# avi2924/Speech-Intent-Recognizer

Measured on AMD Instinct MI355X. Metric: utterances/sec (16 kHz, 3 s clips), inference: HIP STFT+mel+CNN/BiGRU forward + argmax, higher is better.
Workload: dtype f32

## Files before the change

devtools/kernel_ab/legacy_kernels.h:

```cpp
#pragma once
#include "../csrc/bf16x6_kernels.h"

constexpr int XB_ROW = 80;

constexpr int conv_bf16x6_row_bytes(int PC, bool pad = true) {
    const int slots = (4 * PC + 2) * 3;
    return (pad ? slots + ((4 - slots % 8) + 8) % 8 : slots) * 16;
}
constexpr size_t conv_bf16x6_lds_bytes(int PR, int PC, bool pad = true) { return (size_t)3 * (8 * PR + 2) * conv_bf16x6_row_bytes(PC, pad); }


static __global__ __launch_bounds__(256) void gemm_nt_bf16x6_kernel(
    const unsigned short* __restrict__ Ap, const unsigned short* __restrict__ Bp0, const unsigned short* __restrict__ Bp1,
    const float* __restrict__ bias0, const float* __restrict__ bias1, float* __restrict__ C, int ldc, int M, int N, int K) {
    __shared__ __attribute__((aligned(16))) unsigned char As[3 * GB_M * XB_ROW];
    __shared__ __attribute__((aligned(16))) unsigned char Bs[3 * GB_N * XB_ROW];
    const int z = blockIdx.z;
    const unsigned short* __restrict__ Bp = z ? Bp1 : Bp0;
    const float* __restrict__ bias = z ? bias1 : bias0;
    const int m0 = blockIdx.y * GB_M, n0 = blockIdx.x * GB_N;
    const int tid = threadIdx.x, lane = tid & 63, wv = tid >> 6;
    const int wm = wv >> 1, wn = wv & 1, m = lane & 31, h = lane >> 5;
    const size_t planeA = (size_t)M * K, planeB = (size_t)N * K;

// ... 227 lines not shown
                    if (PYb + q < Hp) out[(((size_t)b * Hp + PYb + q) * Wp + PX) * COUT + co] = pooled[q];
            } else {
                float* o = out + ((size_t)b * Wp + PX) * (COUT * Hp) + (size_t)co * Hp + PYb;
                if ((Hp & 3) == 0) {
                    *reinterpret_cast<float4*>(o) = make_float4(pooled[0], pooled[1], pooled[2], pooled[3]);
                } else {
#pragma unroll
                    for (int q = 0; q < 4; ++q)
                        if (PYb + q < Hp) o[q] = pooled[q];
                }
            }
        }
    }
}

static __global__ __launch_bounds__(256) void split3_kernel(const float* __restrict__ in, int ld_in, unsigned short* __restrict__ out,
                                                             size_t rows, int K) {
    split3_rows(in, ld_in, out, rows, K, (size_t)blockIdx.x * 256 + threadIdx.x, (size_t)gridDim.x * 256);
}


constexpr int G3_BM = 160, G3_BN = 256, G3_BK = 32;
constexpr int G3_APLANE = G3_BM * 64, G3_BPLANE = G3_BN * 64;
constexpr int G3_BOFF = 3 * G3_APLANE;
constexpr int G3_STAGE = G3_BOFF + 3 * G3_BPLANE;
constexpr int G3_LDS_BYTES = 2 * G3_STAGE;
constexpr int G3_APIECES = 3 * G3_BM / 16, G3_PIECES = G3_APIECES + 3 * G3_BN / 16;
constexpr int G3_DEFAULT = 16;

template <int KNOCK = G3_DEFAULT>
static __global__ __launch_bounds__(512) void gemm_nt_bf16x6_v3_kernel(
    const unsigned short* __restrict__ Ap, const unsigned short* __restrict__ Bp0, const unsigned short* __restrict__ Bp1,
    const float* __restrict__ bias0, const float* __restrict__ bias1, float* __restrict__ C, int ldc, int M, int N, int K) {
    extern __shared__ __attribute__((aligned(1024))) unsigned char g3_smem[];
    const int nwg = gridDim.x, orig = blockIdx.x, xcd = orig & 7, q = nwg >> 3, rem = nwg & 7;
    const int wgid = (xcd < rem ? xcd * (q + 1) : rem * (q + 1) + (xcd - rem) * q) + (orig >> 3);
    const int nbd = N / G3_BN, nb = 2 * nbd;
    const int mblk = wgid / nb, nbk = wgid - mblk * nb, z = nbk / nbd;
    const int m0 = mblk * G3_BM, n0 = (nbk - z * nbd) * G3_BN;
    const unsigned short* __restrict__ Bp = z ? Bp1 : Bp0;
    const float* __restrict__ bias = z ? bias1 : bias0;
    const int tid = threadIdx.x, lane = tid & 63, wv = tid >> 6, m = lane & 31, h = lane >> 5;
    const size_t planeA = (size_t)M * K, planeB = (size_t)N * K;

    const int lr = lane >> 2;
    const int csrc = (lane & 3) ^ ((lr >> 2) & 3);
    unsigned int poff[10];
#pragma unroll
    for (int i = 0; i < 10; ++i) {
        const int g = wv + 8 * i;
        if (g < G3_APIECES) {
            const int pl = g / 10, rg = g - pl * 10;
            int row = m0 + rg * 16 + lr;
            row = row < M ? row : M - 1;
            poff[i] = (unsigned int)(pl * planeA + (size_t)row * K + csrc * 8);
        } else {
            const int gb = g - G3_APIECES, pl = gb >> 4, rg = gb & 15;
            poff[i] = (unsigned int)(pl * planeB + (size_t)(n0 + rg * 16 + lr) * K + csrc * 8);
        }
    }
    auto piece = [&](int i, int kt, int buf) {
        if (KNOCK & 1) return;
        const int g = wv + 8 * i;
        if (g < G3_PIECES) {
            const unsigned short* src = (g < G3_APIECES ? Ap : Bp) + poff[i] + (size_t)kt * G3_BK;
            __builtin_amdgcn_global_load_lds((sir_gptr_t)src, (sir_lptr_t)(g3_smem + buf * G3_STAGE + g * 1024), 16, 0, 0);
        }
    };
    auto stage = [&](int kt, int buf) {
#pragma unroll
        for (int i = 0; i < 10; ++i) piece(i, kt, buf);
    };

    f32x16 acc[5];
#pragma unroll
    for (int mt = 0; mt < 5; ++mt)
#pragma unroll
        for (int r = 0; r < 16; ++r) acc[mt][r] = 0.0f;

    int fo[2];
#pragma unroll
    for (int ks = 0; ks < 2; ++ks) fo[ks] = m * 64 + ((((ks << 1) | h) ^ ((m >> 2) & 3)) << 4);

    constexpr int SPREAD = (KNOCK >> 3) & 3;
    constexpr bool PREF = (KNOCK >> 5) & 1;
    const int nk = K / G3_BK;
    bf16x8 a[2][3][5], bb[2][3];
    auto read_frags = [&](int buf, int ks) {
        const unsigned char* abase = g3_smem + buf * G3_STAGE;
        const unsigned char* bbase = abase + G3_BOFF + wv * 2048;
#pragma unroll
        for (int p = 0; p < 3; ++p) {
            bb[ks][p] = __builtin_bit_cast(bf16x8, *reinterpret_cast<const uint4*>(bbase + p * G3_BPLANE + fo[ks]));
#pragma unroll
            for (int mt = 0; mt < 5; ++mt)
                a[ks][p][mt] = __builtin_bit_cast(bf16x8, *reinterpret_cast<const uint4*>(abase + p * G3_APLANE + mt * 2048 + fo[ks]));
        }
    };
    auto compute = [&](int buf, int ktn) {
        const int ktl = ktn < nk ? ktn : nk - 1;
        read_frags(buf, 0);
        if (PREF) {
            read_frags(buf, 1);
            __builtin_amdgcn_sched_barrier(0);
        }
#pragma unroll
        for (int ks = 0; ks < 2; ++ks) {
            if (!PREF && ks == 1) read_frags(buf, 1);
            constexpr int PA[6] = {2, 0, 1, 1, 0, 0}, PB[6] = {0, 2, 1, 0, 1, 0};
#pragma unroll
            for (int t = 0; t < 6; ++t)
#pragma unroll
                for (int mt = 0; mt < 5; ++mt) {
                    if (KNOCK & 4) acc[mt][0] += __builtin_bit_cast(float4, a[ks][PA[t]][mt]).x * __builtin_bit_cast(float4, bb[ks][PB[t]]).x;
                    else acc[mt] = __builtin_amdgcn_mfma_f32_32x32x16_bf16(a[ks][PA[t]][mt], bb[ks][PB[t]], acc[mt], 0, 0, 0);
                    const int idx = t * 5 + mt;
                    if (SPREAD && idx % 3 == 2) {
                        if (SPREAD == 1 && ks == 0) piece(idx / 3, ktl, buf ^ 1);
                        if (SPREAD == 2 && ks == (wv >> 2)) piece(idx / 3, ktl, buf ^ 1);
                    }
                }
        }
    };

    stage(0, 0);
    for (int kt = 0; kt < nk; ++kt) {
        __syncthreads();
        if (SPREAD == 0 && kt + 1 < nk) stage(kt + 1, (kt + 1) & 1);
        compute(kt & 1, kt + 1);
    }

    const int n = n0 + wv * 32 + m;
    const float bv = bias ? bias[n] : 0.0f;
    float* crow = C + (size_t)(m0 + 4 * h) * ldc + (size_t)z * N + n;
    if (m0 + G3_BM <= M) {
#pragma unroll
        for (int mt = 0; mt < 5; ++mt)
#pragma unroll
            for (int r = 0; r < 16; ++r) crow[(size_t)(mt * 32 + (r & 3) + 8 * (r >> 2)) * ldc] = acc[mt][r] + bv;
    } else {
#pragma unroll
        for (int mt = 0; mt < 5; ++mt)
#pragma unroll
            for (int r = 0; r < 16; ++r) {
                const int ro = mt * 32 + (r & 3) + 8 * (r >> 2);
                if (m0 + 4 * h + ro < M) crow[(size_t)ro * ldc] = acc[mt][r] + bv;
            }
    }
}

static inline bool gemm_bf16x6_v3_ok(int M, int N, int K) {
    return N % G3_BN == 0 && K % G3_BK == 0 && (size_t)3 * M * K < ((size_t)1 << 31) && (size_t)3 * N * K < ((size_t)1 << 31);
}
```

speech-intent-recognizer_amd/csrc/model_infer.hip:

```cpp
#include "f16x3_kernels.h"
#include "conv_fwd.h"
#include "infer_tables.h"

extern "C" size_t sir_model_workspace_bytes(const sir_handle* h, int batch, int t_frames, int train) {
    (void)h;
    if (train) return sir_train_workspace_bytes_impl(batch, t_frames);
    Dims d;
    if (!make_dims(batch, t_frames, &d)) return 0;
    size_t off[WS_COUNT];
    return iws_layout(d, off);
}

extern "C" int sir_model_workspace_offsets(const sir_handle* h, int batch, int t_frames, int train, size_t* offsets,
                                           int n) {
    (void)h; (void)train;
    Dims d;
    if (!make_dims(batch, t_frames, &d) || !offsets) {
        sir_set_error("sir_model_workspace_offsets: bad shape batch=%d t_frames=%d (need " SIR_SHAPE_LIMITS ")", batch, t_frames);
        return SIR_EINVAL;
    }
    size_t off[WS_COUNT];
    iws_layout(d, off);
    for (int i = 0; i < n && i < WS_COUNT; ++i) offsets[i] = off[i];
    return WS_COUNT;
}

extern "C" int sir_model_infer_table_offsets(const sir_handle* h, int batch, int t_frames, size_t* offsets, int n) {
    (void)h;
    Dims d;
    if (!make_dims(batch, t_frames, &d) || !offsets) {
        sir_set_error("sir_model_infer_table_offsets: bad shape batch=%d t_frames=%d (need " SIR_SHAPE_LIMITS ")", batch, t_frames);
        return SIR_EINVAL;
    }
    const ITabs t = itab_layout(d);
    const size_t v[] = {t.e0, t.d1, t.d3, t.rows, t.tab2, t.tab3, t.record, t.nonfinite, t.count, (size_t)WS_PAD};
    const int nv = (int)(sizeof(v) / sizeof(v[0]));
    for (int i = 0; i < n && i < nv; ++i) offsets[i] = v[i];
    return nv;
}

static int model_infer_impl(const char* who, sir_handle* h, const sir_model_weights* w, const float* feats, const int32_t* frames, int batch,
                            int t_frames, float* logits, int64_t* argmax, void* workspace, size_t workspace_bytes, void* stream_) {
    if (!h || !w || !feats || !logits || !workspace) { sir_set_error("%s: NULL argument", who); return SIR_EINVAL; }
    Dims d;
    if (!make_dims(batch, t_frames, &d)) {
        sir_set_error("%s: unsupported shape batch=%d t_frames=%d (need " SIR_SHAPE_LIMITS ")", who, batch, t_frames);
        return SIR_EINVAL;
    }
    if (h->cfg.n_mels != 64) { sir_set_error("%s: the model is wired for 64 mels (models.py:23)", who); return SIR_EUNSUPPORTED; }
    if (w->num_classes < 1 || w->num_classes > 64) { sir_set_error("%s: num_classes=%d", who, w->num_classes); return SIR_EINVAL; }
    size_t off[WS_COUNT];
    const size_t need = iws_layout(d, off);
    if (workspace_bytes < need) { sir_set_error("%s: workspace %zu < %zu", who, workspace_bytes, need); return SIR_ENOMEM; }
    if (((uintptr_t)workspace & 255) != 0) { sir_set_error("%s: workspace must be 256-byte aligned", who); return SIR_EINVAL; }
    const bool ragged = frames != nullptr;
    hipStream_t st = (hipStream_t)stream_;
    const IPtrs p = carve(workspace, off, d);
    const ITabPtrs& t = p.t;
    const int B = d.B, S = d.S;
    const bool proj_throughput = h->cluster_multi;

    const SirConvPlan cp = sir_conv_plan(&d, true);
    const bool w2 = cp.fwd_wino;
    const int BT = w2 ? B + 1 : B;

    const long long prep_key = ((long long)B << 32) | (unsigned)d.T;
    sir_handle::PrepEntry* pe = nullptr;
    for (auto& e : h->prep)
        if (e.ws == workspace) pe = &e;
    const bool reuse_prep = pe && h->weights_version != 0 && pe->version == h->weights_version && pe->key == prep_key;
    if (!reuse_prep) {
        SirProfScope prof(h, SIR_K_PREP, st);
        const int bn_c[3] = {32, 64, 128}, bn_o[3] = {0, 32, 96};
        for (int i = 0; i < 3; ++i)
            hipLaunchKernelGGL(prep_bn_kernel, dim3(1), dim3(128), 0, st, w->bn_w[i], w->bn_b[i], w->bn_mean[i], w->bn_var[i],
                               p.bns + bn_o[i], p.bnt + bn_o[i], bn_c[i], i == 0 ? w->conv_w[0] : (const float*)nullptr, i == 0 ? 288 : 0, h->status);
        for (int i = 0; i < 4; ++i) sir_prep_whh_quad(h, st, w->gru_w_hh[i], p.whh[i]);
        if (w2) hipLaunchKernelGGL(prep_conv_w_wino_f16x3_kernel, dim3(prep_blocks(WCB_W2)), dim3(256), 0, st, w->conv_w[1], p.wcb2, 32, 64, h->status);
        else hipLaunchKernelGGL(prep_conv_w_wino_bf16x3_kernel, dim3(prep_blocks(WCB_W2)), dim3(256), 0, st, w->conv_w[1], p.wcb2, 32, 64);
        if (w2) hipLaunchKernelGGL(prep_conv_w_wino_f16x3_kernel, dim3(prep_blocks(WCB_W3)), dim3(256), 0, st, w->conv_w[2], p.wcb3, 64, 128, h->status);
        else hipLaunchKernelGGL(prep_conv_w_wino_bf16x3_kernel, dim3(prep_blocks(WCB_W3)), dim3(256), 0, st, w->conv_w[2], p.wcb3, 64, 128);
        hipLaunchKernelGGL(prep_conv_w_bf16x3_kernel, dim3(prep_blocks(WCB_W3_TAPS)), dim3(256), 0, st, w->conv_w[2], p.wcb3d, 64, 128);
        for (int dir = 0; dir < 2; ++dir) {
            hipLaunchKernelGGL(split2h_weights_kernel, dim3(WS_DIR0_BLOCKS), dim3(256), 0, st, w->gru_w_ih[dir], 1024, p.wsl0[dir], (size_t)768, 1024, h->status);
            hipLaunchKernelGGL(split2h_weights_kernel, dim3(WS_DIR1_BLOCKS), dim3(256), 0, st, w->gru_w_ih[2 + dir], 512, p.wsl1[dir], (size_t)768, 512, h->status);
        }
        if (!pe) { pe = &h->prep[h->prep_next]; h->prep_next = (h->prep_next + 1) % 4; }
        pe->ws = workspace; pe->version = h->weights_version; pe->key = prep_key;
    }
    SIR_KCHECK();

    {
        SirProfScope prof(h, SIR_K_CONV1, st);
        hipLaunchKernelGGL(pad_extent_kernel, dim3(B), dim3(256), 0, st, feats, d.T, ragged ? nullptr : t.e0, (const int*)frames, t.nonfinite);
        if (ragged) {
            hipLaunchKernelGGL(ragged_tables_kernel, dim3(1), dim3(1024), 0, st, (const int*)frames, d, t.e0, t.d1, t.d3, t.tab2, t.tab3, t.rows, h->status);
            hipLaunchKernelGGL(conv1_mfma_bn_relu_pool_ragged_kernel, conv1_grid(B, d.wp1), dim3(256), 0, st, feats,
                               w->conv_w[0], p.bns, p.bnt, p.a1, 64, d.T, 32, d.wp1, t.d1, t.e0);
            if (!w2) hipLaunchKernelGGL(ragged_mask_kernel, dim3(32, B), dim3(256), 0, st, p.a1, t.e0, 1, 32, d.wp1, 32);
        } else {
            if (w2) hipLaunchKernelGGL(pad_tables_kernel, dim3(1), dim3(1024), 0, st, t.e0, d, t.d1, t.d3, t.tab2, t.tab3, t.rows, p.xz);
            hipLaunchKernelGGL(conv1_mfma_bn_relu_pool_kernel, conv1_grid(BT, d.wp1), dim3(256), 0, st, feats,
                               w->conv_w[0], p.bns, p.bnt, p.a1, 64, d.T, 32, d.wp1, p.xz, B, w2 ? t.d1 : nullptr);
        }
    }
    {
        SirProfScope prof(h, SIR_K_CONV2, st);
        if (ragged) {
            SIR_TRY((conv_fwd<32, 64, 0, true>(h, st, w2, cp.geo2, B, p.a1, p.wcb2, nullptr, p.bns + 32, p.bnt + 32, p.a2, nullptr, t.tab2, (B + 1) * d.k2max,
                                               t.e0, 1)));
            if (!w2) hipLaunchKernelGGL(ragged_mask_kernel, dim3(16, B), dim3(256), 0, st, p.a2, t.e0, 2, 16, d.wp2, 64);
        } else
            SIR_TRY((conv_fwd<32, 64, 0>(h, st, w2, cp.geo2, BT, p.a1, p.wcb2, nullptr, p.bns + 32, p.bnt + 32, p.a2, nullptr, t.tab2, (B + 1) * d.k2max)));
    }
    {
        SirProfScope prof(h, SIR_K_CONV3, st);
        if (ragged)
            SIR_TRY((conv_fwd<64, 128, 1, true>(h, st, w2, cp.geo3, B, p.a2, p.wcb3, p.wcb3d, p.bns + 96, p.bnt + 96, p.x0, (float2*)p.xs, t.tab3, (B + 1) * d.k3max,
                                                t.e0, 2)));
        else
            SIR_TRY((conv_fwd<64, 128, 1>(h, st, w2, cp.geo3, BT, p.a2, p.wcb3, p.wcb3d, p.bns + 96, p.bnt + 96, p.x0, (float2*)p.xs, t.tab3, (B + 1) * d.k3max)));
    }
    SIR_KCHECK();

    const int M = B * S;
    const int* const nlive0 = w2 || ragged ? t.d3 : nullptr;
    const int* const nlive1 = ragged ? t.d3 : nullptr;
    {
        SirProfScope prof(h, SIR_K_GEMM_IH0, st);
        if (w2 || ragged)
            SIR_TRY(launch_gemm_nt_f16x3_gather(h, st, p.xs, p.wsl0[0], p.wsl0[1], w->gru_b_ih[0], w->gru_b_ih[1], p.gi, 1536,
                                                t.rows, BT * S, 768, 1024, proj_throughput, t.record));
        else
            SIR_TRY(launch_gemm_nt_f16x3(h, st, p.xs, p.wsl0[0], p.wsl0[1], w->gru_b_ih[0], w->gru_b_ih[1], p.gi, 1536, M, 768, 1024));
    }
    {
        SirProfScope prof(h, SIR_K_GRU0, st);
        SIR_TRY(sir_launch_gru_quad(h, st, false, p.gi, w->gru_w_hh[0], w->gru_w_hh[1], w->gru_b_hh[0], w->gru_b_hh[1], p.y0, B, S, nullptr,
                                    p.xs, p.whh[0], p.whh[1], nlive0, ragged));
    }
    {
        SirProfScope prof(h, SIR_K_GEMM_IH1, st);
        if (ragged)
            SIR_TRY(launch_gemm_nt_f16x3_gather(h, st, p.xs, p.wsl1[0], p.wsl1[1], w->gru_b_ih[2], w->gru_b_ih[3], p.gi, 1536,
                                                t.rows, M, 768, 512, proj_throughput, t.record));
        else
            SIR_TRY(launch_gemm_nt_f16x3(h, st, p.xs, p.wsl1[0], p.wsl1[1], w->gru_b_ih[2], w->gru_b_ih[3], p.gi, 1536, M, 768, 512));
    }
    {
        SirProfScope prof(h, SIR_K_GRU1, st);
        SIR_TRY(sir_launch_gru_quad(h, st, false, p.gi, w->gru_w_hh[2], w->gru_w_hh[3], w->gru_b_hh[2], w->gru_b_hh[3], p.y1, B, S, nullptr,
                                    nullptr, p.whh[2], p.whh[3], nlive1, ragged));
    }
    SIR_KCHECK();

    {
        SirProfScope prof(h, SIR_K_ATTN, st);
        if (ragged)
            hipLaunchKernelGGL(attention_pool_ragged_kernel, dim3(B), dim3(256), 0, st, p.y1, w->attn_w, w->attn_b, p.ctx, S, w->fc_w, w->fc_b,
                               w->num_classes, logits, (long long*)argmax, t.d3, t.nonfinite);
        else
            hipLaunchKernelGGL(attention_pool_kernel, dim3(B), dim3(256), 0, st, p.y1, w->attn_w, w->attn_b, p.ctx, S, w->fc_w, w->fc_b,
                               w->num_classes, logits, (long long*)argmax, t.nonfinite, nullptr);
    }
    SIR_KCHECK();
    return SIR_OK;
}

extern "C" int sir_model_infer(sir_handle* h, const sir_model_weights* w, const float* feats, int batch, int t_frames,
                               float* logits, int64_t* argmax, void* workspace, size_t workspace_bytes, void* stream_) {
    return model_infer_impl("sir_model_infer", h, w, feats, nullptr, batch, t_frames, logits, argmax, workspace, workspace_bytes, stream_);
}

extern "C" int sir_model_infer_ragged(sir_handle* h, const sir_model_weights* w, const float* feats, const int32_t* frames, int batch,
                                      int t_frames, float* logits, int64_t* argmax, void* workspace, size_t workspace_bytes,
                                      void* stream_) {
    if (!frames) { sir_set_error("sir_model_infer_ragged: NULL frames"); return SIR_EINVAL; }
    return model_infer_impl("sir_model_infer_ragged", h, w, feats, frames, batch, t_frames, logits, argmax, workspace, workspace_bytes, stream_);
}
```

speech-intent-recognizer_amd/csrc/model_kernels.h:

```cpp
#pragma once
#include "sir_internal.h"
#include "model_shape.h"

typedef float f32x16 __attribute__((ext_vector_type(16)));
typedef float mk_f32x2 __attribute__((ext_vector_type(2)));

#define SIR_BN_EPS 1e-5f


constexpr unsigned int SIR_STATUS_BN_PARAM = 8192u;
__device__ __forceinline__ bool sir_finite(float v) { return fabsf(v) < INFINITY; }
__device__ __forceinline__ void sir_flag_bn_param(bool ok, unsigned int* status) {
    if (!ok) __hip_atomic_fetch_or(status, SIR_STATUS_BN_PARAM, __ATOMIC_RELAXED, __HIP_MEMORY_SCOPE_AGENT);
}

#ifndef SIR_NO_STANDALONE_KERNELS
static __global__ void prep_bn_kernel(const float* __restrict__ g, const float* __restrict__ b, const float* __restrict__ mean,
                               const float* __restrict__ var, float* __restrict__ scale, float* __restrict__ shift, int c,
                               const float* __restrict__ w1, int n1, unsigned int* __restrict__ status) {
    const int i = blockIdx.x * blockDim.x + threadIdx.x;
    if (i >= c) return;
    const float s = g[i] / sqrtf(var[i] + SIR_BN_EPS);
    const float t = b[i] - mean[i] * s;
    scale[i] = s;
    shift[i] = t;
    bool ok = sir_finite(s) && sir_finite(t);
    for (int j = i; j < n1; j += c) ok = ok && sir_finite(w1[j]);
    sir_flag_bn_param(ok, status);
}
#endif

constexpr int C1_PROWS = 4, C1_PCOLS = 32;
constexpr int C1_TR = 2 * C1_PROWS + 2, C1_TC = 2 * C1_PCOLS + 2;
inline dim3 conv1_grid(int images, int Wp) { return dim3(images, 1, (Wp + C1_PCOLS - 1) / C1_PCOLS); }

#ifndef SIR_NO_STANDALONE_KERNELS
template <bool RAGGED>
__device__ __forceinline__ void conv1_mfma_bn_relu_pool_body(
    const float* __restrict__ x, const float* __restrict__ w, const float* __restrict__ scale,
    const float* __restrict__ shift, float* __restrict__ out, int H, int W, int Hp, int Wp,
    const float* __restrict__ xtail, int nx, const int* __restrict__ lim, const int* __restrict__ xlim) {
    __shared__ float tiles[2][C1_TR * C1_TC];
    const int b = blockIdx.x, px0 = blockIdx.z * C1_PCOLS;
    const int wlim = lim ? min(Wp, lim[b]) : Wp;
    if (px0 >= wlim) return;
    const int tid = threadIdx.x, lane = tid & 63, wv = tid >> 6, j = lane & 31, kh = lane >> 5;
    const float* xb = b < nx ? x + (size_t)b * H * W : xtail;
    const int Wx = RAGGED ? min(W, xlim[b]) : W;
    constexpr int NPRE = (C1_TR * C1_TC + 255) / 256;
    float pre[NPRE];
    auto fetch = [&](int py0) {
#pragma unroll
        for (int q = 0; q < NPRE; ++q) {
            const int i = tid + 256 * q, ty = i / C1_TC, tx = i - ty * C1_TC;
            const int gy = 2 * py0 - 1 + ty, gx = 2 * px0 - 1 + tx;
            pre[q] = (i < C1_TR * C1_TC && gy >= 0 && gy < H && gx >= 0 && gx < Wx) ? xb[(size_t)gy * W + gx] : 0.0f;
        }
    };
    fetch(0);
    float wa[5];
    int boff[5];
#pragma unroll
    for (int s = 0; s < 5; ++s) {
        const int tap = 2 * s + kh;
        wa[s] = tap < 9 ? w[j * 9 + tap] : 0.0f;
        const int tc = tap < 9 ? tap : 8;
        boff[s] = (tc / 3) * C1_TC + (tc % 3) + j;
    }
    float sc[16], sh[16];
#pragma unroll
    for (int r = 0; r < 16; ++r) {
        const int ch = (r & 3) + 8 * (r >> 2) + 4 * kh;
        sc[r] = scale[ch]; sh[r] = shift[ch];
    }
    const bool odd = j & 1;
    int it = 0;
    for (int py0 = 0; py0 < Hp; py0 += C1_PROWS, ++it) {
        float* tile = tiles[it & 1];
#pragma unroll
        for (int q = 0; q < NPRE; ++q)
            if (tid + 256 * q < C1_TR * C1_TC) tile[tid + 256 * q] = pre[q];
        __syncthreads();
        if (py0 + C1_PROWS < Hp) fetch(py0 + C1_PROWS);
        const int py = py0 + wv;
        if (py >= Hp) continue;
        const float* trow = tile + (2 * wv) * C1_TC;
#pragma unroll
        for (int h = 0; h < 2; ++h) {
            if (px0 + 16 * h >= wlim) break;
            f32x16 acc0, acc1;
#pragma unroll
            for (int r = 0; r < 16; ++r) { acc0[r] = 0.0f; acc1[r] = 0.0f; }
#pragma unroll
            for (int s = 0; s < 5; ++s) {
                const float b0 = trow[boff[s] + 32 * h], b1 = trow[boff[s] + 32 * h + C1_TC];
                acc0 = __builtin_amdgcn_mfma_f32_32x32x2f32(wa[s], b0, acc0, 0, 0, 0);
                acc1 = __builtin_amdgcn_mfma_f32_32x32x2f32(wa[s], b1, acc1, 0, 0, 0);
            }
            float m[16];
#pragma unroll
            for (int r = 0; r < 16; r += 2) {
                const mk_f32x2 s2 = {sc[r], sc[r + 1]}, h2 = {sh[r], sh[r + 1]};
                const mk_f32x2 y0 = __builtin_elementwise_fma((mk_f32x2){acc0[r], acc0[r + 1]}, s2, h2);
                const mk_f32x2 y1 = __builtin_elementwise_fma((mk_f32x2){acc1[r], acc1[r + 1]}, s2, h2);
                const float v0 = fmaxf(y0.x, y1.x), v1 = fmaxf(y0.y, y1.y);
                const float nb0 = __builtin_bit_cast(float, __builtin_amdgcn_update_dpp(0, __builtin_bit_cast(int, v0), 0xB1, 0xF, 0xF, true));
                const float nb1 = __builtin_bit_cast(float, __builtin_amdgcn_update_dpp(0, __builtin_bit_cast(int, v1), 0xB1, 0xF, 0xF, true));
                m[r] = fmaxf(fmaxf(v0, nb0), 0.0f);
                m[r + 1] = fmaxf(fmaxf(v1, nb1), 0.0f);
            }
            const int px = px0 + 16 * h + (j >> 1);
            const float4 lo = odd ? make_float4(m[8], m[9], m[10], m[11]) : make_float4(m[0], m[1], m[2], m[3]);
            const float4 hi = odd ? make_float4(m[12], m[13], m[14], m[15]) : make_float4(m[4], m[5], m[6], m[7]);
            if (px < wlim) {
                float* o = out + (((size_t)b * Hp + py) * Wp + px) * 32 + 4 * kh + (odd ? 16 : 0);
                *reinterpret_cast<float4*>(o) = lo;
                *reinterpret_cast<float4*>(o + 8) = hi;
            }
        }
    }
}
static __global__ __launch_bounds__(256, 4) void conv1_mfma_bn_relu_pool_kernel(
    const float* __restrict__ x, const float* __restrict__ w, const float* __restrict__ scale,
    const float* __restrict__ shift, float* __restrict__ out, int H, int W, int Hp, int Wp,
    const float* __restrict__ xtail, int nx, const int* __restrict__ lim) {
    conv1_mfma_bn_relu_pool_body<false>(x, w, scale, shift, out, H, W, Hp, Wp, xtail, nx, lim, nullptr);
}
static __global__ __launch_bounds__(256, 4) void conv1_mfma_bn_relu_pool_ragged_kernel(
    const float* __restrict__ x, const float* __restrict__ w, const float* __restrict__ scale,
    const float* __restrict__ shift, float* __restrict__ out, int H, int W, int Hp, int Wp,
    const int* __restrict__ lim, const int* __restrict__ xlim) {
    conv1_mfma_bn_relu_pool_body<true>(x, w, scale, shift, out, H, W, Hp, Wp, nullptr, (int)gridDim.x, lim, xlim);
}
#endif

constexpr int GB_M = 128, GB_N = 64, GB_K = 32, GB_S = GB_K + 4;

constexpr int GRU_H = 256, GRU_BW = 2;
constexpr int GRU_NPART = 4;
constexpr int GRU_KPER4 = 64 / GRU_NPART;
constexpr int GRU_KREG4 = 3;
constexpr int GRU_KLDS4 = 2;
constexpr int GRU_KSTR4 = GRU_KPER4 - GRU_KREG4 - GRU_KLDS4;
constexpr int GRU_NQ = (GRU_BW + GRU_NPART - 1) / GRU_NPART;
constexpr int GRU_THREADS = 256 * GRU_NPART;
constexpr size_t GRU_LDS_BYTES =
    (size_t)(GRU_NPART * GRU_KLDS4 * 3 * 256 * 4 + GRU_BW * GRU_H + GRU_NPART * GRU_BW * 3 * GRU_H) * 4;

__device__ __forceinline__ float sigmoidf_(float x) { return 1.0f / (1.0f + expf(-x)); }

template <int NB>
__device__ __forceinline__ void gru_fma4(float (&acc)[NB], const float4 w, const float4 (&h4)[NB]) {
#pragma unroll
    for (int bb = 0; bb < NB; ++bb) {
        acc[bb] = fmaf(w.x, h4[bb].x, acc[bb]); acc[bb] = fmaf(w.y, h4[bb].y, acc[bb]);
        acc[bb] = fmaf(w.z, h4[bb].z, acc[bb]); acc[bb] = fmaf(w.w, h4[bb].w, acc[bb]);
    }
}


#ifndef SIR_NO_STANDALONE_KERNELS
template <bool RAGGED>
__device__ __forceinline__ void attention_pool_body(const float* __restrict__ y, const float* __restrict__ aw,
                                                    const float* __restrict__ ab, float* __restrict__ ctx,
                                                    int SR, const float* __restrict__ fcw,
                                                    const float* __restrict__ fcb, int C,
                                                    float* __restrict__ logits, long long* __restrict__ amax,
                                                    const int* __restrict__ slen, const int* __restrict__ bad_row,
                                                    const double* __restrict__ sumsq) {
    __shared__ float sc[ATT_MAX_S];
    __shared__ float cs[512];
    __shared__ float lg[64];
    const int b = blockIdx.x, tid = threadIdx.x, lane = tid & 63, wv = tid >> 6;
    const int S = RAGGED ? min(SR, slen[b]) : SR;
    bool bad = bad_row && bad_row[b] != 0;
    if (sumsq) bad |= (__double2hiint(sumsq[0]) & 0x7ff00000) == 0x7ff00000;
    if (RAGGED && S < 1) {
        const float qnan = __builtin_nanf("");
        for (int c = tid; c < 512; c += 256) ctx[(size_t)b * 512 + c] = qnan;
        if (logits && tid < C) logits[(size_t)b * C + tid] = qnan;
        if (logits && amax && tid == 0) amax[b] = 0;
        return;
    }
    const float* yb = y + (size_t)b * SR * 512;
    float a[8];
#pragma unroll
    for (int i = 0; i < 8; ++i) a[i] = aw[lane + 64 * i];
    for (int t0 = 4 * wv; t0 < S; t0 += 16) {
        float v[4][8];
#pragma unroll
        for (int k = 0; k < 4; ++k)
#pragma unroll
            for (int i = 0; i < 8; ++i) v[k][i] = (t0 + k < S) ? yb[(size_t)(t0 + k) * 512 + lane + 64 * i] : 0.0f;
#pragma unroll
        for (int k = 0; k < 4; ++k) {
            float d = 0.0f;
#pragma unroll
            for (int i = 0; i < 8; ++i) d = fmaf(v[k][i], a[i], d);
#pragma unroll
            for (int o = 32; o > 0; o >>= 1) d += __shfl_xor(d, o);
            if (lane == 0 && t0 + k < S) sc[t0 + k] = d + ab[0];
        }
    }
    __syncthreads();
    __shared__ float ex[ATT_MAX_S];
    float mx = -INFINITY;
    for (int t = 0; t < S; ++t) mx = fmaxf(mx, sc[t]);
    if (tid < S) ex[tid] = expf(sc[tid] - mx);
    __syncthreads();
    float den = 0.0f;
    for (int t = 0; t < S; ++t) den += ex[t];
    __syncthreads();
    if (tid < S) ex[tid] = ex[tid] / den;
    __syncthreads();
    for (int c = tid; c < 512; c += 256) {
        float acc = 0.0f;
        for (int t = 0; t < S; ++t) acc = fmaf(ex[t], yb[(size_t)t * 512 + c], acc);
        ctx[(size_t)b * 512 + c] = acc;
        cs[c] = acc;
    }
    if (!logits) return;
    __syncthreads();
    for (int j = tid >> 3; j < C; j += 32) {
        const int part = tid & 7;
        const float4* wr = reinterpret_cast<const float4*>(fcw + (size_t)j * 512 + part * 64);
        const float4* cr = reinterpret_cast<const float4*>(cs + part * 64);
        float d = 0.0f;
#pragma unroll
        for (int i = 0; i < 16; ++i) {
            const float4 wv4 = wr[i], c4 = cr[i];
            d = fmaf(c4.x, wv4.x, d); d = fmaf(c4.y, wv4.y, d); d = fmaf(c4.z, wv4.z, d); d = fmaf(c4.w, wv4.w, d);
        }
        d += __shfl_xor(d, 1); d += __shfl_xor(d, 2); d += __shfl_xor(d, 4);
        if (part == 0) {
            d += fcb[j];
            if (bad) d = __builtin_nanf("");
            lg[j] = d;
            logits[(size_t)b * C + j] = d;
        }
    }
    if (!amax) return;
    __syncthreads();
    if (tid == 0) {
        float best = lg[0];
        int bi = 0;
        for (int c = 1; c < C; ++c)
            if (lg[c] > best) { best = lg[c]; bi = c; }
        amax[b] = bi;
    }
}
static __global__ __launch_bounds__(256) void attention_pool_kernel(const float* __restrict__ y, const float* __restrict__ aw,
                                                             const float* __restrict__ ab, float* __restrict__ ctx,
                                                             int S, const float* __restrict__ fcw,
                                                             const float* __restrict__ fcb, int C,
                                                             float* __restrict__ logits, long long* __restrict__ amax,
                                                             const int* __restrict__ bad_row, const double* __restrict__ sumsq) {
    attention_pool_body<false>(y, aw, ab, ctx, S, fcw, fcb, C, logits, amax, nullptr, bad_row, sumsq);
}
static __global__ __launch_bounds__(256) void attention_pool_ragged_kernel(const float* __restrict__ y, const float* __restrict__ aw,
                                                             const float* __restrict__ ab, float* __restrict__ ctx,
                                                             int S, const float* __restrict__ fcw,
                                                             const float* __restrict__ fcb, int C,
                                                             float* __restrict__ logits, long long* __restrict__ amax,
                                                             const int* __restrict__ slen, const int* __restrict__ bad_row) {
    attention_pool_body<true>(y, aw, ab, ctx, S, fcw, fcb, C, logits, amax, slen, bad_row, nullptr);
}
#endif
```

speech-intent-recognizer_amd/csrc/model_train_fwd.hip:

```cpp
#include "f16x3_kernels.h"
#include "train_fwd_kernels.h"
#include "conv_fwd.h"

size_t sir_train_workspace_bytes_impl(int batch, int t_frames) {
    TDims d;
    if (!make_tdims(batch, t_frames, &d)) return 0;
    size_t off[TB_COUNT];
    return tws_layout(d, off);
}

extern "C" int sir_model_train_workspace_offsets(const sir_handle* h, int batch, int t_frames, size_t* offsets, int n) {
    (void)h;
    TDims d;
    if (!make_tdims(batch, t_frames, &d) || !offsets) {
        sir_set_error("sir_model_train_workspace_offsets: bad shape batch=%d t_frames=%d (need " SIR_SHAPE_LIMITS ")", batch, t_frames);
        return SIR_EINVAL;
    }
    size_t off[TB_COUNT];
    tws_layout(d, off);
    for (int i = 0; i < n && i < TB_COUNT; ++i) offsets[i] = off[i];
    return TB_COUNT;
}

extern "C" int sir_model_train_fwd(sir_handle* h, const sir_model_weights* w, float* const bn_running_mean[3],
                                   float* const bn_running_var[3], const float* feats, int batch, int t_frames,
                                   float bn_momentum, float dropout_p, uint64_t dropout_seed, float* logits, void* workspace, size_t workspace_bytes, void* stream_) {
    return sir_model_train_fwd_cfg(h, w, bn_running_mean, bn_running_var, feats, batch, t_frames, bn_momentum, dropout_p, dropout_seed,
                                   nullptr, logits, workspace, workspace_bytes, stream_);
}

static int train_fwd_impl(const char* who, sir_handle* h, const sir_model_weights* w, float* const bn_running_mean[3],
                          float* const bn_running_var[3], const float* feats, const int32_t* frames, int batch, int t_frames,
                          float bn_momentum, float dropout_p, uint64_t dropout_seed, const sir_train_config* cfg,
                          float* logits, void* workspace, size_t workspace_bytes, void* stream_) {
    const bool ragged = frames != nullptr;
    TDims d;
    size_t off[TB_COUNT];
    int rc = check_common(who, h, w, batch, t_frames, workspace, workspace_bytes, &d, off);
    if (rc != SIR_OK) return rc;
    if (!feats || !logits || !bn_running_mean || !bn_running_var) { sir_set_error("%s: NULL argument", who); return SIR_EINVAL; }
    for (int i = 0; ragged && i < 3; ++i)
        if (!bn_running_mean[i] || !bn_running_var[i]) { sir_set_error("%s: NULL running statistics", who); return SIR_EINVAL; }
    if (dropout_p < 0.0f || dropout_p >= 1.0f) { sir_set_error("%s: dropout_p=%f", who, dropout_p); return SIR_EINVAL; }
    hipStream_t st = (hipStream_t)stream_;
    TPtrs p = carve(workspace, off);
    const int B = d.B, S = d.S, T = d.T;
    const RagPtrs rg = rag_ptrs(p.rag, B);
    float *scale = p.bn, *shift = p.bn + 224, *smean = p.bn + 448, *sinv = p.bn + 672;

    const SirConvPlan& cp = d.conv;
    const bool w2 = cp.fwd_wino;
    {
        SirProfScope prof(h, SIR_K_T_PREP, st);
        PrepJobs pj{};
        int nj = 0, blocks = 0;
        auto add = [&](PrepKind kind, const float* src, void* dst, int a, int b, int nblk) {
            pj.kind[nj] = kind; pj.src[nj] = src; pj.dst[nj] = dst; pj.a[nj] = a; pj.b[nj] = b; pj.block0[nj] = blocks;
            blocks += nblk; ++nj;
        };
        pj.status = h->status;
        add(w2 ? PREP_CONV_W_WINO_F16X3 : PREP_CONV_W_WINO_BF16X3, w->conv_w[1], p.wcb2, 32, 64, prep_blocks(WCB_W2));
        add(w2 ? PREP_CONV_W_WINO_F16X3 : PREP_CONV_W_WINO_BF16X3, w->conv_w[2], p.wcb3, 64, 128, prep_blocks(WCB_W3));
        if (!w2) add(PREP_CONV_W_BF16X3, w->conv_w[2], p.wcb3d, 64, 128, prep_blocks(WCB_W3_TAPS));
        if (cp.dgrad2_wino) add(PREP_CONV_WT_WINO_F16X3, w->conv_w[1], p.wcb2t, 32, 64, prep_blocks(WCB_W2));
        else add(PREP_CONV_WT_BF16X3, w->conv_w[1], p.wcb2t, 32, 64, prep_blocks(WCB_W2_TAPS));
        add(cp.dgrad3_wino ? PREP_CONV_WT_WINO_F16X3 : PREP_CONV_WT_WINO_BF16X3, w->conv_w[2], p.wcb3t, 64, 128, prep_blocks(WCB_W3));
        for (int dir = 0; dir < 2; ++dir) {
            add(PREP_SPLIT2H, w->gru_w_ih[dir], p.wsl0 + dir * WS_DIR0, 1024, 768, WS_DIR0_BLOCKS);
            add(PREP_SPLIT2H, w->gru_w_ih[2 + dir], p.wsl1 + dir * WS_DIR1, 512, 768, WS_DIR1_BLOCKS);
        }
        for (int i = 0; i < 4; ++i) {
            add(PREP_WHH_QUAD, w->gru_w_hh[i], (char*)p.wht + (size_t)i * GRU_FRAG_BYTES, 0, 0, GQ_FRAG_THREADS / 256);
            add(PREP_WHH_BWD_QUAD, w->gru_w_hh[i], (char*)p.wr4 + (size_t)i * GRU_FRAG_BYTES, 0, 0, BQ_FRAG_THREADS / 256);
        }
        pj.block0[nj] = blocks;
        pj.njobs = nj;
        static_assert(PREP_MAX_JOBS >= 18, "job table");
        hipLaunchKernelGGL(train_prep_kernel, dim3(blocks), dim3(256), 0, st, pj);
    }
    SIR_KCHECK();

    {   SirProfScope prof(h, SIR_K_T_CONV1, st);
        if (cfg->bn_frozen[0]) {
            hipLaunchKernelGGL(bn_fold_running_kernel, dim3(1), dim3(64), 0, st, w->bn_w[0], w->bn_b[0], (const float*)bn_running_mean[0],
                               (const float*)bn_running_var[0], 32, scale, shift, smean, sinv, w->conv_w[0], 288, h->status);
        } else {
            const int tiles = d.c1gx * d.c1gy;
            int per_img = (2048 + B - 1) / B;
            per_img = per_img < 1 ? 1 : (per_img > tiles ? tiles : per_img);
            hipLaunchKernelGGL(conv1_moments_kernel, dim3(per_img, B), dim3(256), 0, st, feats, (float*)p.stats, 64, T, d.c1gx, d.c1gy);
            hipLaunchKernelGGL(conv1_moments_reduce_kernel, dim3(C1_NMOM), dim3(256), 0, st, (const float*)p.stats, per_img * B, p.c1m);
            hipLaunchKernelGGL(conv1_bn_from_moments_kernel, dim3(1), dim3(64), 0, st, (const double*)p.c1m, w->conv_w[0],
                               (double)B * 64 * T, w->bn_w[0], w->bn_b[0], bn_running_mean[0], bn_running_var[0], bn_momentum, scale, shift, smean, sinv, h->status);
        }
        if (ragged) {
            hipLaunchKernelGGL(ragged_widths_kernel, dim3((B + 255) / 256), dim3(256), 0, st, (const int*)frames, B, T, p.rag, h->status);
            hipLaunchKernelGGL(conv1_mfma_bn_relu_pool_ragged_kernel, conv1_grid(B, d.wp1), dim3(256), 0, st,
                               feats, w->conv_w[0], scale, shift, p.a1, 64, T, 32, d.wp1, rg.w1, rg.fw);
            hipLaunchKernelGGL(ragged_zero_tail_kernel, dim3(32, B), dim3(256), 0, st, p.a1, rg.w1, 32, d.wp1, 32, 1);
        } else
            hipLaunchKernelGGL(conv1_mfma_bn_relu_pool_kernel, conv1_grid(B, d.wp1), dim3(256), 0, st,
                               feats, w->conv_w[0], scale, shift, p.a1, 64, T, 32, d.wp1, (const float*)nullptr, B, (const int*)nullptr);
    }
    {
        {   SirProfScope prof(h, SIR_K_T_CONV2, st);
            SIR_TRY((conv_fwd<32, 64, 2>(h, st, w2, cp.geo2, B, p.a1, p.wcb2, nullptr, nullptr, nullptr, p.z2, p.stats)));
        }
        SirProfScope prof(h, SIR_K_T_BN2, st);
        if (cfg->bn_frozen[1])
            hipLaunchKernelGGL(bn_fold_running_kernel, dim3(1), dim3(64), 0, st, w->bn_w[1], w->bn_b[1], (const float*)bn_running_mean[1],
                               (const float*)bn_running_var[1], 64, scale + 32, shift + 32, smean + 32, sinv + 32, (const float*)nullptr, 0, h->status);
        else
            hipLaunchKernelGGL(bn_finalize_kernel, dim3(64), dim3(256), 0, st, (const float2*)p.stats, w2 ? (int)wino2_stat_blocks(B, 32, d.wp1, h->num_cus) : d.c2wx * B, 64,
                               (double)B * 32 * d.wp1, w->bn_w[1], w->bn_b[1], bn_running_mean[1], bn_running_var[1], bn_momentum,
                               scale + 32, shift + 32, smean + 32, sinv + 32, h->status);
        if (ragged)
            hipLaunchKernelGGL((bn_relu_pool_kernel<false, true>), dim3(grid_for((size_t)B * 16 * d.wp2 * 16)), dim3(256), 0, st, p.z2,
                               scale + 32, shift + 32, p.a2, B, 32, d.wp1, 64, 16, d.wp2, 256.0f, h->status, rg.w2);
        else
            hipLaunchKernelGGL(bn_relu_pool_kernel<false>, dim3(grid_for((size_t)B * 16 * d.wp2 * 16)), dim3(256), 0, st, p.z2,
                               scale + 32, shift + 32, p.a2, B, 32, d.wp1, 64, 16, d.wp2, 256.0f, h->status, (const int*)nullptr);
    }
    {
        {   SirProfScope prof(h, SIR_K_T_CONV3, st);
            SIR_TRY((conv_fwd<64, 128, 2>(h, st, w2, cp.geo3, B, p.a2, p.wcb3, p.wcb3d, nullptr, nullptr, p.z3, p.stats)));
        }
        SirProfScope prof(h, SIR_K_T_BN3, st);
        if (cfg->bn_frozen[2])
            hipLaunchKernelGGL(bn_fold_running_kernel, dim3(1), dim3(128), 0, st, w->bn_w[2], w->bn_b[2], (const float*)bn_running_mean[2],
                               (const float*)bn_running_var[2], 128, scale + 96, shift + 96, smean + 96, sinv + 96, (const float*)nullptr, 0, h->status);
        else
            hipLaunchKernelGGL(bn_finalize_kernel, dim3(128), dim3(256), 0, st, (const float2*)p.stats, w2 ? (int)wino2_stat_blocks(B, 16, d.wp2, h->num_cus) : d.c3fx * B, 128,
                               (double)B * 16 * d.wp2, w->bn_w[2], w->bn_b[2], bn_running_mean[2], bn_running_var[2], bn_momentum,
                               scale + 96, shift + 96, smean + 96, sinv + 96, h->status);
        if (ragged)
            hipLaunchKernelGGL((bn_relu_pool_kernel<true, true>), dim3(grid_for((size_t)B * 8 * d.wp3 * 32)), dim3(256), 0, st, p.z3,
                               scale + 96, shift + 96, p.x0, B, 16, d.wp2, 128, 8, d.wp3, 512.0f, h->status, rg.sb);
        else
            hipLaunchKernelGGL(bn_relu_pool_kernel<true>, dim3(grid_for((size_t)B * 8 * d.wp3 * 32)), dim3(256), 0, st, p.z3,
                               scale + 96, shift + 96, p.x0, B, 16, d.wp2, 128, 8, d.wp3, 512.0f, h->status, (const int*)nullptr);
    }
    SIR_KCHECK();

    const int M = B * S;
    {   SirProfScope prof(h, SIR_K_T_GEMM_IH0, st);
        hipLaunchKernelGGL(split2h_kernel, dim3(2048), dim3(256), 0, st, (const float*)p.x0, 1024, p.xs, (size_t)M, 1024);
        SIR_TRY(launch_gemm_nt_f16x3(h, st, (const unsigned short*)p.xs, (const unsigned short*)p.wsl0,
                                     (const unsigned short*)(p.wsl0 + WS_DIR0), w->gru_b_ih[0], w->gru_b_ih[1], p.gi, 1536, M, 768, 1024));
    }
    {   SirProfScope prof(h, SIR_K_T_GRU0, st);
        if (ragged) hipLaunchKernelGGL(ragged_zero_tail_kernel, dim3(S, B), dim3(256), 0, st, p.y0, rg.sb, S, 512, 1, 0);
        SIR_TRY(sir_launch_gru_quad(h, st, true, p.gi, w->gru_w_hh[0], w->gru_w_hh[1], w->gru_b_hh[0], w->gru_b_hh[1], p.y0, B, S, p.g0, nullptr,
                                    (const char*)p.wht, (const char*)p.wht + GRU_FRAG_BYTES, ragged ? rg.sb : nullptr, ragged));
    }
    const float* y0in = p.y0;
    {   SirProfScope prof(h, SIR_K_T_GEMM_IH1, st);
        if (dropout_p > 0.0f) {
            hipLaunchKernelGGL(dropout_split2h_kernel, dim3(2048), dim3(256), 0, st, (const float*)p.y0, p.y0d, p.xs, (size_t)M * 512,
                               dropout_p, (unsigned long long)dropout_seed);
            y0in = p.y0d;
        } else {
            hipLaunchKernelGGL(split2h_kernel, dim3(2048), dim3(256), 0, st, y0in, 512, p.xs, (size_t)M, 512);
        }
        SIR_TRY(launch_gemm_nt_f16x3(h, st, (const unsigned short*)p.xs, (const unsigned short*)p.wsl1,
                                     (const unsigned short*)(p.wsl1 + WS_DIR1), w->gru_b_ih[2], w->gru_b_ih[3], p.gi, 1536, M, 768, 512));
    }
    {   SirProfScope prof(h, SIR_K_T_GRU1, st);
        if (ragged) hipLaunchKernelGGL(ragged_zero_tail_kernel, dim3(S, B), dim3(256), 0, st, p.y1, rg.sb, S, 512, 1, 0);
        SIR_TRY(sir_launch_gru_quad(h, st, true, p.gi, w->gru_w_hh[2], w->gru_w_hh[3], w->gru_b_hh[2], w->gru_b_hh[3], p.y1, B, S, p.g1, nullptr,
                                    (const char*)p.wht + 2 * GRU_FRAG_BYTES, (const char*)p.wht + 3 * GRU_FRAG_BYTES, ragged ? rg.sb : nullptr, ragged));
    }
    SirProfScope prof_head(h, SIR_K_T_HEAD, st);
    if (ragged) {
        hipLaunchKernelGGL(attention_pool_ragged_kernel, dim3(B), dim3(256), 0, st, p.y1, w->attn_w, w->attn_b, p.ctx, S, w->fc_w,
                           w->fc_b, w->num_classes, logits, (long long*)nullptr, rg.sb, (const int*)nullptr);
        SIR_KCHECK();
        return SIR_OK;
    }
    hipLaunchKernelGGL(attention_pool_kernel, dim3(B), dim3(256), 0, st, p.y1, w->attn_w, w->attn_b, p.ctx, S, w->fc_w,
                       w->fc_b, w->num_classes, logits, (long long*)nullptr, (const int*)nullptr,
                       cfg->bn_frozen[0] ? (const double*)nullptr : (const double*)p.c1m + c1_r_index(4, 4));
    SIR_KCHECK();
    return SIR_OK;
}

extern "C" int sir_model_train_fwd_cfg(sir_handle* h, const sir_model_weights* w, float* const bn_running_mean[3],
                                       float* const bn_running_var[3], const float* feats, int batch, int t_frames,
                                       float bn_momentum, float dropout_p, uint64_t dropout_seed, const sir_train_config* cfg,
                                       float* logits, void* workspace, size_t workspace_bytes, void* stream_) {
    return train_fwd_impl("sir_model_train_fwd", h, w, bn_running_mean, bn_running_var, feats, nullptr, batch, t_frames, bn_momentum, dropout_p,
                          dropout_seed, cfg ? cfg : &kTrainAllLive, logits, workspace, workspace_bytes, stream_);
}

extern "C" int sir_model_train_fwd_ragged(sir_handle* h, const sir_model_weights* w, const float* const bn_running_mean[3],
                                          const float* const bn_running_var[3], const float* feats, const int32_t* frames, int batch,
                                          int t_frames, float dropout_p, uint64_t dropout_seed, const sir_train_config* cfg,
                                          float* logits, void* workspace, size_t workspace_bytes, void* stream_) {
    if (!cfg || !cfg->bn_frozen[0] || !cfg->bn_frozen[1] || !cfg->bn_frozen[2]) {
        sir_set_error("sir_model_train_fwd_ragged: lengths (frames per clip) need every BatchNorm on its frozen running statistics "
                      "(bn_frozen = {1, 1, 1}): with batch statistics a clip has no result of its own");
        return SIR_EUNSUPPORTED;
    }
    if (!frames) { sir_set_error("sir_model_train_fwd_ragged: NULL frames"); return SIR_EINVAL; }
    return train_fwd_impl("sir_model_train_fwd_ragged", h, w, (float* const*)bn_running_mean, (float* const*)bn_running_var, feats, frames,
                          batch, t_frames, 0.0f, dropout_p, dropout_seed, cfg, logits, workspace, workspace_bytes, stream_);
}
```

Measured before the change: 771,500.

## Split conv1 row walk across blocks with single-tile 16-row strips

The conv1 kernel no longer walks all pooled rows of an image in one block with a double-buffered prefetch loop. It now launches a grid dimension over 16-row strips, and each block loads one larger LDS tile once, syncs once, and has its four waves cover the strip's rows. The goal is more blocks in flight and fewer serialized load/sync rounds per block. The cost is recomputing halo rows between strips, a bigger LDS tile that may lower occupancy, and no overlap of load with compute. The old walk kernel is kept in devtools as a legacy A/B variant, along with debug timestamp hooks.

```diff
diff --git a/devtools/kernel_ab/legacy_kernels.h b/devtools/kernel_ab/legacy_kernels.h
--- a/devtools/kernel_ab/legacy_kernels.h
+++ b/devtools/kernel_ab/legacy_kernels.h
@@ -403,3 +403,123 @@
 static inline bool gemm_bf16x6_v3_ok(int M, int N, int K) {
     return N % G3_BN == 0 && K % G3_BK == 0 && (size_t)3 * M * K < ((size_t)1 << 31) && (size_t)3 * N * K < ((size_t)1 << 31);
 }
+
+
+static __device__ long long c1w8_dbg_stamps[8][8];
+template <bool RAGGED, int DBG = 0>
+__device__ __forceinline__ void conv1_mfma_bn_relu_pool_walk8_body(
+    const float* __restrict__ x, const float* __restrict__ w, const float* __restrict__ scale,
+    const float* __restrict__ shift, float* __restrict__ out, int H, int W, int Hp, int Wp,
+    const float* __restrict__ xtail, int nx, const int* __restrict__ lim, const int* __restrict__ xlim) {
+    __shared__ float tiles[2][C1_TR * C1_TC];
+    __shared__ long long stamps[DBG ? 64 : 1];
+    const int b = blockIdx.x, px0 = blockIdx.z * C1_PCOLS;
+    const int wlim = lim ? min(Wp, lim[b]) : Wp;
+    if (px0 >= wlim) return;
+    const int tid = threadIdx.x, lane = tid & 63, wv = tid >> 6, j = lane & 31, kh = lane >> 5;
+    const bool stamper = DBG && blockIdx.x == 0 && blockIdx.z == 0 && tid == 0;
+    auto stamp = [&](int round, int k) {
+        if (DBG) {
+            asm volatile("" ::: "memory");
+            if (stamper && round < 8) stamps[8 * round + k] = __builtin_amdgcn_s_memtime();
+            asm volatile("" ::: "memory");
+        }
+    };
+    const float* xb = b < nx ? x + (size_t)b * H * W : xtail;
+    const int Wx = RAGGED ? min(W, xlim[b]) : W;
+    constexpr int NPRE = (C1_TR * C1_TC + 255) / 256;
+    float pre[NPRE];
+    auto fetch = [&](int py0) {
+#pragma unroll
+        for (int q = 0; q < NPRE; ++q) {
+            const int i = tid + 256 * q, ty = i / C1_TC, tx = i - ty * C1_TC;
+            const int gy = 2 * py0 - 1 + ty, gx = 2 * px0 - 1 + tx;
+            pre[q] = (i < C1_TR * C1_TC && gy >= 0 && gy < H && gx >= 0 && gx < Wx) ? xb[(size_t)gy * W + gx] : 0.0f;
+        }
+    };
+    fetch(0);
+    float wa[5];
+    int boff[5];
+#pragma unroll
+    for (int s = 0; s < 5; ++s) {
+        const int tap = 2 * s + kh;
+        wa[s] = tap < 9 ? w[j * 9 + tap] : 0.0f;
+        const int tc = tap < 9 ? tap : 8;
+        boff[s] = (tc / 3) * C1_TC + (tc % 3) + j;
+    }
+    float sc[16], sh[16];
+#pragma unroll
+    for (int r = 0; r < 16; ++r) {
+        const int ch = (r & 3) + 8 * (r >> 2) + 4 * kh;
+        sc[r] = scale[ch]; sh[r] = shift[ch];
+    }
+    const bool odd = j & 1;
+    int it = 0;
+    for (int py0 = 0; py0 < Hp; py0 += C1_PROWS, ++it) {
+        stamp(it, 0);
+        float* tile = tiles[it & 1];
+#pragma unroll
+        for (int q = 0; q < NPRE; ++q)
+            if (tid + 256 * q < C1_TR * C1_TC) tile[tid + 256 * q] = pre[q];
+        stamp(it, 1);
+        __syncthreads();
+        stamp(it, 2);
+        if (py0 + C1_PROWS < Hp) fetch(py0 + C1_PROWS);
+        stamp(it, 3);
+        const int py = py0 + wv;
+        if (py >= Hp) continue;
+        const float* trow = tile + (2 * wv) * C1_TC;
+#pragma unroll
+        for (int h = 0; h < 2; ++h) {
+            if (px0 + 16 * h >= wlim) break;
+            f32x16 acc0, acc1;
+#pragma unroll
+            for (int r = 0; r < 16; ++r) { acc0[r] = 0.0f; acc1[r] = 0.0f; }
+#pragma unroll
+            for (int s = 0; s < 5; ++s) {
+                const float b0 = trow[boff[s] + 32 * h], b1 = trow[boff[s] + 32 * h + C1_TC];
+                acc0 = __builtin_amdgcn_mfma_f32_32x32x2f32(wa[s], b0, acc0, 0, 0, 0);
+                acc1 = __builtin_amdgcn_mfma_f32_32x32x2f32(wa[s], b1, acc1, 0, 0, 0);
+            }
+            if (DBG) asm volatile("v_mov_b32 %0, %0" : "+v"(acc1[15]));
+            stamp(it, 4 + 2 * h);
+            float m[16];
+#pragma unroll
+            for (int r = 0; r < 16; r += 2) {
+                const mk_f32x2 s2 = {sc[r], sc[r + 1]}, h2 = {sh[r], sh[r + 1]};
+                const mk_f32x2 y0 = __builtin_elementwise_fma((mk_f32x2){acc0[r], acc0[r + 1]}, s2, h2);
+                const mk_f32x2 y1 = __builtin_elementwise_fma((mk_f32x2){acc1[r], acc1[r + 1]}, s2, h2);
+                const float v0 = fmaxf(y0.x, y1.x), v1 = fmaxf(y0.y, y1.y);
+                const float nb0 = __builtin_bit_cast(float, __builtin_amdgcn_update_dpp(0, __builtin_bit_cast(int, v0), 0xB1, 0xF, 0xF, true));
+                const float nb1 = __builtin_bit_cast(float, __builtin_amdgcn_update_dpp(0, __builtin_bit_cast(int, v1), 0xB1, 0xF, 0xF, true));
+                m[r] = fmaxf(fmaxf(v0, nb0), 0.0f);
+                m[r + 1] = fmaxf(fmaxf(v1, nb1), 0.0f);
+            }
+            const int px = px0 + 16 * h + (j >> 1);
+            const float4 lo = odd ? make_float4(m[8], m[9], m[10], m[11]) : make_float4(m[0], m[1], m[2], m[3]);
+            const float4 hi = odd ? make_float4(m[12], m[13], m[14], m[15]) : make_float4(m[4], m[5], m[6], m[7]);
+            if (px < wlim) {
+                float* o = out + (((size_t)b * Hp + py) * Wp + px) * 32 + 4 * kh + (odd ? 16 : 0);
+                *reinterpret_cast<float4*>(o) = lo;
+                *reinterpret_cast<float4*>(o + 8) = hi;
+            }
+            stamp(it, 5 + 2 * h);
+        }
+    }
+    if (DBG && stamper)
+        for (int k = 0; k < 64; ++k) c1w8_dbg_stamps[k >> 3][k & 7] = stamps[k];
+}
+inline dim3 conv1_walk8_grid(int images, int Wp) { return dim3(images, 1, (Wp + C1_PCOLS - 1) / C1_PCOLS); }
+template <int DBG>
+static __global__ __launch_bounds__(256, 4) void conv1_mfma_bn_relu_pool_walk8_kernel(
+    const float* __restrict__ x, const float* __restrict__ w, const float* __restrict__ scale,
+    const float* __restrict__ shift, float* __restrict__ out, int H, int W, int Hp, int Wp,
+    const float* __restrict__ xtail, int nx, const int* __restrict__ lim) {
+    conv1_mfma_bn_relu_pool_walk8_body<false, DBG>(x, w, scale, shift, out, H, W, Hp, Wp, xtail, nx, lim, nullptr);
+}
+static __global__ __launch_bounds__(256, 4) void conv1_mfma_bn_relu_pool_walk8_ragged_kernel(
+    const float* __restrict__ x, const float* __restrict__ w, const float* __restrict__ scale,
+    const float* __restrict__ shift, float* __restrict__ out, int H, int W, int Hp, int Wp,
+    const int* __restrict__ lim, const int* __restrict__ xlim) {
+    conv1_mfma_bn_relu_pool_walk8_body<true>(x, w, scale, shift, out, H, W, Hp, Wp, nullptr, (int)gridDim.x, lim, xlim);
+}
diff --git a/speech-intent-recognizer_amd/csrc/model_infer.hip b/speech-intent-recognizer_amd/csrc/model_infer.hip
--- a/speech-intent-recognizer_amd/csrc/model_infer.hip
+++ b/speech-intent-recognizer_amd/csrc/model_infer.hip
@@ -95,12 +95,12 @@
         hipLaunchKernelGGL(pad_extent_kernel, dim3(B), dim3(256), 0, st, feats, d.T, ragged ? nullptr : t.e0, (const int*)frames, t.nonfinite);
         if (ragged) {
             hipLaunchKernelGGL(ragged_tables_kernel, dim3(1), dim3(1024), 0, st, (const int*)frames, d, t.e0, t.d1, t.d3, t.tab2, t.tab3, t.rows, h->status);
-            hipLaunchKernelGGL(conv1_mfma_bn_relu_pool_ragged_kernel, conv1_grid(B, d.wp1), dim3(256), 0, st, feats,
+            hipLaunchKernelGGL(conv1_mfma_bn_relu_pool_ragged_kernel, conv1_grid(B, 32, d.wp1), dim3(256), 0, st, feats,
                                w->conv_w[0], p.bns, p.bnt, p.a1, 64, d.T, 32, d.wp1, t.d1, t.e0);
             if (!w2) hipLaunchKernelGGL(ragged_mask_kernel, dim3(32, B), dim3(256), 0, st, p.a1, t.e0, 1, 32, d.wp1, 32);
         } else {
             if (w2) hipLaunchKernelGGL(pad_tables_kernel, dim3(1), dim3(1024), 0, st, t.e0, d, t.d1, t.d3, t.tab2, t.tab3, t.rows, p.xz);
-            hipLaunchKernelGGL(conv1_mfma_bn_relu_pool_kernel, conv1_grid(BT, d.wp1), dim3(256), 0, st, feats,
+            hipLaunchKernelGGL(conv1_mfma_bn_relu_pool_kernel, conv1_grid(BT, 32, d.wp1), dim3(256), 0, st, feats,
                                w->conv_w[0], p.bns, p.bnt, p.a1, 64, d.T, 32, d.wp1, p.xz, B, w2 ? t.d1 : nullptr);
         }
     }
diff --git a/speech-intent-recognizer_amd/csrc/model_kernels.h b/speech-intent-recognizer_amd/csrc/model_kernels.h
--- a/speech-intent-recognizer_amd/csrc/model_kernels.h
+++ b/speech-intent-recognizer_amd/csrc/model_kernels.h
@@ -32,32 +32,41 @@
 
 constexpr int C1_PROWS = 4, C1_PCOLS = 32;
 constexpr int C1_TR = 2 * C1_PROWS + 2, C1_TC = 2 * C1_PCOLS + 2;
-inline dim3 conv1_grid(int images, int Wp) { return dim3(images, 1, (Wp + C1_PCOLS - 1) / C1_PCOLS); }
+constexpr int C1_SPROWS = 16;
+inline dim3 conv1_grid(int images, int Hp, int Wp) { return dim3(images, (Hp + C1_SPROWS - 1) / C1_SPROWS, (Wp + C1_PCOLS - 1) / C1_PCOLS); }
 
 #ifndef SIR_NO_STANDALONE_KERNELS
-template <bool RAGGED>
+static __device__ long long c1_dbg_stamps[16];
+template <bool RAGGED, int SPROWS = C1_SPROWS, int DBG = 0>
 __device__ __forceinline__ void conv1_mfma_bn_relu_pool_body(
     const float* __restrict__ x, const float* __restrict__ w, const float* __restrict__ scale,
     const float* __restrict__ shift, float* __restrict__ out, int H, int W, int Hp, int Wp,
     const float* __restrict__ xtail, int nx, const int* __restrict__ lim, const int* __restrict__ xlim) {
-    __shared__ float tiles[2][C1_TR * C1_TC];
-    const int b = blockIdx.x, px0 = blockIdx.z * C1_PCOLS;
+    constexpr int NST = (2 * SPROWS + 2) * C1_TC, NPRE = (NST + 255) / 256;
+    __shared__ float tile[NST];
+    const int b = blockIdx.x, py0 = blockIdx.y * SPROWS, px0 = blockIdx.z * C1_PCOLS;
     const int wlim = lim ? min(Wp, lim[b]) : Wp;
     if (px0 >= wlim) return;
     const int tid = threadIdx.x, lane = tid & 63, wv = tid >> 6, j = lane & 31, kh = lane >> 5;
+    const bool stamper = DBG && blockIdx.x == 0 && blockIdx.y == 0 && blockIdx.z == 0 && tid == 0;
+    auto stamp = [&](int k) {
+        if (DBG) {
+            asm volatile("" ::: "memory");
+            if (stamper && k < 16) c1_dbg_stamps[k] = __builtin_amdgcn_s_memtime();
+            asm volatile("" ::: "memory");
+        }
+    };
+    stamp(0);
     const float* xb = b < nx ? x + (size_t)b * H * W : xtail;
     const int Wx = RAGGED ? min(W, xlim[b]) : W;
-    constexpr int NPRE = (C1_TR * C1_TC + 255) / 256;
     float pre[NPRE];
-    auto fetch = [&](int py0) {
-#pragma unroll
-        for (int q = 0; q < NPRE; ++q) {
-            const int i = tid + 256 * q, ty = i / C1_TC, tx = i - ty * C1_TC;
-            const int gy = 2 * py0 - 1 + ty, gx = 2 * px0 - 1 + tx;
-            pre[q] = (i < C1_TR * C1_TC && gy >= 0 && gy < H && gx >= 0 && gx < Wx) ? xb[(size_t)gy * W + gx] : 0.0f;
-        }
-    };
-    fetch(0);
+#pragma unroll
+    for (int q = 0; q < NPRE; ++q) {
+        const int i = tid + 256 * q, ty = i / C1_TC, tx = i - ty * C1_TC;
+        const int gy = 2 * py0 - 1 + ty, gx = 2 * px0 - 1 + tx;
+        pre[q] = (i < NST && gy >= 0 && gy < H && gx >= 0 && gx < Wx) ? xb[(size_t)gy * W + gx] : 0.0f;
+    }
+    stamp(1);
     float wa[5];
     int boff[5];
 #pragma unroll
@@ -74,17 +83,16 @@
         sc[r] = scale[ch]; sh[r] = shift[ch];
     }
     const bool odd = j & 1;
-    int it = 0;
-    for (int py0 = 0; py0 < Hp; py0 += C1_PROWS, ++it) {
-        float* tile = tiles[it & 1];
-#pragma unroll
-        for (int q = 0; q < NPRE; ++q)
-            if (tid + 256 * q < C1_TR * C1_TC) tile[tid + 256 * q] = pre[q];
-        __syncthreads();
-        if (py0 + C1_PROWS < Hp) fetch(py0 + C1_PROWS);
-        const int py = py0 + wv;
-        if (py >= Hp) continue;
-        const float* trow = tile + (2 * wv) * C1_TC;
+#pragma unroll
+    for (int q = 0; q < NPRE; ++q)
+        if (tid + 256 * q < NST) tile[tid + 256 * q] = pre[q];
+    stamp(2);
+    __syncthreads();
+    stamp(3);
+    for (int r0 = wv; r0 < SPROWS; r0 += 4) {
+        const int py = py0 + r0;
+        if (py >= Hp) break;
+        const float* trow = tile + (2 * r0) * C1_TC;
 #pragma unroll
         for (int h = 0; h < 2; ++h) {
             if (px0 + 16 * h >= wlim) break;
@@ -118,6 +126,7 @@
                 *reinterpret_cast<float4*>(o + 8) = hi;
             }
         }
+        stamp(4 + (r0 >> 2));
     }
 }
 static __global__ __launch_bounds__(256, 4) void conv1_mfma_bn_relu_pool_kernel(
diff --git a/speech-intent-recognizer_amd/csrc/model_train_fwd.hip b/speech-intent-recognizer_amd/csrc/model_train_fwd.hip
--- a/speech-intent-recognizer_amd/csrc/model_train_fwd.hip
+++ b/speech-intent-recognizer_amd/csrc/model_train_fwd.hip
@@ -95,11 +95,11 @@
         }
         if (ragged) {
             hipLaunchKernelGGL(ragged_widths_kernel, dim3((B + 255) / 256), dim3(256), 0, st, (const int*)frames, B, T, p.rag, h->status);
-            hipLaunchKernelGGL(conv1_mfma_bn_relu_pool_ragged_kernel, conv1_grid(B, d.wp1), dim3(256), 0, st,
+            hipLaunchKernelGGL(conv1_mfma_bn_relu_pool_ragged_kernel, conv1_grid(B, 32, d.wp1), dim3(256), 0, st,
                                feats, w->conv_w[0], scale, shift, p.a1, 64, T, 32, d.wp1, rg.w1, rg.fw);
             hipLaunchKernelGGL(ragged_zero_tail_kernel, dim3(32, B), dim3(256), 0, st, p.a1, rg.w1, 32, d.wp1, 32, 1);
         } else
-            hipLaunchKernelGGL(conv1_mfma_bn_relu_pool_kernel, conv1_grid(B, d.wp1), dim3(256), 0, st,
+            hipLaunchKernelGGL(conv1_mfma_bn_relu_pool_kernel, conv1_grid(B, 32, d.wp1), dim3(256), 0, st,
                                feats, w->conv_w[0], scale, shift, p.a1, 64, T, 32, d.wp1, (const float*)nullptr, B, (const int*)nullptr);
     }
     {
```

Result: no change. 771,400 (median of 2 runs) (-0.0%).
